# zqs01/ASR_chinese_e2e

Measured on AMD Instinct MI355X. Metric: training throughput (utterances/s; frames/s = x T), AISHELL-1-shaped 80-mel T=500, higher is better.
Workload: dtype bf16; 1 GPU; configs[2]: joint CTC/attention (lambda=0.3) encoder-decoder, bf16, per-GPU batch 32, T=500, F=80, V=4232, 6 layers, d_model 512, 8x64 heads, ff 1024, dropout 0.0, fwd+loss+CER+bwd+clip+Noam/Adam per step, eager launches; global_batch=32, seq_len=500, parallelism=dp1

## Files before the change

### asr_chinese_e2e_amd/Models/transformer_official.py

```python
import contextlib
import math

import numpy as np
import torch

from .. import engine as E
from .. import kernels as K
from ..Bases import BaseConfig, BaseModel
from ..Utils import Pack

SOS_ID, EOS_ID, PAD_ID = 2, 3, 0
PE_MAXLEN = 5000
CLIP_NORM = 5.0


def mwer_settings(weight, nbest, beam, frame_topk, blank_skip):
    try:
        ok = not isinstance(weight, (bool, str)) and math.isfinite(float(weight)) and float(weight) >= 0.0
    except (TypeError, ValueError):
        ok = False
    if not ok:
        raise ValueError(f"mwer_weight={weight!r}: a finite number >= 0 (0 = no MWER term)")
    for name, v in (("mwer_nbest", nbest), ("mwer_beam", beam), ("mwer_frame_topk", frame_topk)):
        if isinstance(v, bool) or not isinstance(v, (int, np.integer)):
# ... 676 lines not shown
            al = self._align_lists(ctc_logits(), wave_len, ids, alignable=ok, confidence=confidence)
            for o, a in zip(out, al):
                o["tokens"] = a["tokens"]
                if confidence is not None:
                    o["confidence"] = a["confidence"]
        return out

    def _ctc_cer(self, logits, wave_len, labels32, lab_len):
        ids, lens = K.ctc_greedy_decode(logits, wave_len, PAD_ID)
        return self._cer_ids(ids, labels32, hyp_len=lens, ref_len=lab_len)

    def train_step(self, input, loss_scale=1.0, count_hook=None):
        eng, x, wave_len, prep = self._prepare(input, training=self.training)
        B, T, _ = x.shape
        lam = self.ctc_weight
        ys_in, ys_out, labels32, dec_len, lab_len, n_valid = prep
        pending = count_hook(n_valid, B) if count_hook is not None else None
        zero, self._zero_lazy = (self._flat.g if getattr(self, "_zero_lazy", False) else None), False
        eng.refresh_transposes(zero=zero)
        enc, ecache = self.encode(eng, x, wave_len, training=True)
        batch_div = None
        if pending is not None:
            n_valid, batch_div = pending.wait()
        row_nll = nll = None
        d_enc = None
        pg = None
        ctc_done = None
        ctc_scale = dict(grad_scale=lam * loss_scale, grad_scale_div=batch_div) if batch_div is not None else dict(grad_scale=lam * loss_scale / float(B))
        ctc_async = (self.use_decoder and self.use_ctc and eng._aux_active() and not eng.deterministic)
        if self.use_decoder:
            cross_len, Tk = self._cross(eng, input, wave_len, T)
        if ctc_async:
            eng.decoder_kv_async(prep, enc, B, T, Tk)
            nll, d_enc, ctc_done = eng.ctc_branch_async(enc, wave_len, labels32, lab_len, B, T, **ctc_scale)
        if self.use_decoder:
            pred, dcache = eng.decoder_fwd(prep, enc, cross_len, B, T, Tk)
            ids = torch.empty(ys_out.shape, dtype=torch.int32, device=pred.device) if self.cer_in_iterate else None
            w_ce = (1.0 - lam) if self.use_ctc else 1.0
            row_nll, dpred = K.xent_fwd_bwd(pred, ys_out.reshape(-1), n_valid, PAD_ID, smoothing=self.label_smoothing, grad_scale=w_ce * loss_scale, dlogits=pred,
                                            argmax=ids)
            if ids is not None:
                pg = (ids, ys_out)
        if self.use_ctc and not ctc_async:
            path = torch.empty(B, T, dtype=torch.int32, device=enc.device) if (self.cer_in_iterate and not self.use_decoder) else None
            mwer = {}
            if self.mwer_weight > 0.0:
                mwer = dict(mwer_grad_scale=self.mwer_weight * loss_scale / (1.0 if batch_div is not None else float(B)))
            nll, d_enc = eng.ctc_fwd_bwd(enc, wave_len, labels32, lab_len, B, T, best_path=path, **ctc_scale, **mwer)
            if path is not None:
                def score():
                    ids, lens = K.ctc_collapse(path, wave_len, PAD_ID)
                    return self._cer_ids(ids, labels32, hyp_len=lens, ref_len=lab_len)
                pg = self._cer_beside_backward(eng, score, (path, wave_len, labels32, lab_len), inline=lambda: (score(), None))
        if self.use_decoder:
            if d_enc is None:
                d_enc = torch.zeros_like(enc)
            eng.decoder_bwd(dcache, dpred, d_enc, d_enc_ready=ctc_done)
            if pg is not None:
                pg = self._cer_beside_backward(eng, lambda: self._cer_ids(ids, ys_out), pg, inline=lambda: pg)
        eng.encoder_bwd(ecache, d_enc)
        loss = K.loss_combine(row_nll, n_valid, nll, (1.0 - lam) if self.use_ctc else 1.0, lam)
        self._mwer_mean = None
        if self.mwer_weight > 0.0 and self.use_ctc and not ctc_async:
            risk = eng.last_mwer[4]
            self._mwer_mean = risk.sum() / (batch_div[0] if batch_div is not None else float(B))
            loss = loss.clone()
            loss[0] += self.mwer_weight * self._mwer_mean
        return loss, pg

    def mwer_risk(self, input, nbest=None, beam_size=None, frame_topk=None, blank_skip=None):
        d = self._mwer
        _, m = mwer_settings(0.0, d["nbest"] if nbest is None else nbest, d["beam"] if beam_size is None else beam_size,
                             d["frame_topk"] if frame_topk is None else frame_topk, blank_skip)
        if blank_skip is None:
            m["thr"] = d["thr"]
        if self.use_decoder or not self.use_ctc:
            raise ValueError("mwer_risk needs the CTC-only model (TransformerCTC)")
        eng = self._ensure_engine(input.wave.device)
        was_training, eng.training = eng.training, False
        try:
            with torch.no_grad():
                out = self.forward(input)
        finally:
            eng.training = was_training
        logits = out.ctc_logits.contiguous()
        B, T, V = logits.shape
        wave_len = input.wave_len.to(torch.int32).contiguous()
        prep = K.dec_preprocess(input.tgt_for_input.contiguous(), SOS_ID, EOS_ID)
        labels32, lab_len = prep[2], prep[4]
        vals, ids, blank_lp = K.ctc_frame_topk(logits.view(B * T, V), min(m["frame_topk"], V), PAD_ID)
        search_len = wave_len
        if m["thr"] is not None:
            vals, ids, blank_lp, search_len, _ = K.ctc_blank_skip_compact(vals, ids, blank_lp, wave_len, m["thr"], B, T)
        Lh = min(T, K.MWER_MAX_LEN, 2 * labels32.shape[1] + 8)
        tok, ln, _ = K.ctc_prefix_beam(vals, ids, blank_lp, search_len, B, T, m["beam"], m["nbest"], PAD_ID, max_len=Lh)
        res = K.ctc_mwer(logits, wave_len, tok, ln, labels32, lab_len, blank=PAD_ID, want_grad=False)
        tok, ln, err, post, risk = (t.cpu().tolist() for t in (tok, ln, res["err"], res["post"], res["risk"]))
        return [{"risk": risk[b], "errors": [err[b][r] for r in range(m["nbest"]) if ln[b][r] >= 0],
                 "posteriors": [post[b][r] for r in range(m["nbest"]) if ln[b][r] >= 0],
                 "nbest": [tok[b][r][:min(ln[b][r], Lh)] for r in range(m["nbest"]) if ln[b][r] >= 0]} for b in range(B)]

    def iterate(self, input, optimizer=None, is_train=True):
        if optimizer is None or not is_train:
            with torch.no_grad():
                output = self.forward(input)
                return self.cal_metrics(output, input), None
        if self._ema_active:
            raise RuntimeError("iterate(is_train=True) inside ema_weights(): the parameters are swapped with their average")
        self._ensure_engine(input.wave.device)
        optimizer.zero_grad()
        if getattr(optimizer, "fused_step", None) is None or not getattr(optimizer, "keeps_grad_views", False):
            self._grads_checked = False
        self.zero_flat_grads()
        loss, pg = self.train_step(input)
# ... 59 lines not shown
```

### asr_chinese_e2e_amd/_lib.py

```python
import ctypes
import os
from ctypes import c_char_p, c_float, c_int, c_size_t, c_uint32, c_void_p

import torch

_HERE = os.path.dirname(os.path.abspath(__file__))
LIB_PATH = os.environ.get("ASR_HIP_LIB") or os.path.join(_HERE, "libasr_hip.so")

ASR_F32, ASR_BF16 = 0, 1
ACT_NONE, ACT_RELU, ACT_RELU_MASK = 0, 1, 2
ABI_VERSION = 10
DROP_PRE, DROP_POST = 1, 2
SPEED_TILE = 1024
RESAMPLE_TILE = 1024
REVERB_TILE, REVERB_CHUNK, REVERB_MAX_TAPS = 1024, 256, 8192
REVERB_FFT_N, REVERB_FFT_MAX_TAPS = 4096, 65536
NOISE_MIX_TILE = 4096
VAD_CTX_MAX = 1024
ALIGN_LONG_MAX_LABELS = 8192
SPECAUG_MAX_RANGES = 8
KWS_MAX_LEN, KWS_MAX_KEYWORDS, KWS_MAX_CAP = 16, 65536, 64
EDIT_LDS_DIR_BYTES, EDIT_MAX_REF = 98304, 16384
EDIT_COR, EDIT_SUB, EDIT_DEL, EDIT_INS = 0, 1, 2, 3
NBEST_MAX_N, NBEST_MAX_LEN, NBEST_MAX_ALTS, NBEST_EPS = 64, 256, 8, -1
RESCORE_MAX_N, RESCORE_MAX_K, RESCORE_MAX_G, RESCORE_MAX_U = 64, 8, 65536, 1 << 20
MWER_MAX_N, MWER_MAX_LEN, MWER_ABSENT, MWER_LONG = 16, 255, 1, 2
STREAM_OPEN = 0x3fffffff

P, I, F, Z, U = c_void_p, c_int, c_float, c_size_t, c_uint32

class TnProblem(ctypes.Structure):
    _fields_ = [("dY", P), ("X", P), ("dW", P), ("dbias", P), ("M", I), ("N", I), ("K", I), ("ldy", I), ("ldx", I), ("ldw", I)]


TN_GROUP_MAX = 8


class LnReduceItem(ctypes.Structure):
    _fields_ = [("ws", P), ("dgamma", P), ("dbeta", P), ("dbias", P), ("rows", I)]


LN_REDUCE_MAX = 16


class DecLayerPlan(ctypes.Structure):
    _fields_ = ([(n, I) for n in ("B", "To", "T", "d", "H", "dk", "ff")] + [("drop_p", F), ("seed", U * 5), ("ld_kv_c_T", I)] +
                [(n, P) for n in ("dec_len", "cross_len",
                                  "w_qkv_s", "w_fc_s", "w_q_c", "w_fc_c", "w_1", "w_2",
                                  "b_qkv_s", "b_fc_s", "b_q_c", "b_fc_c", "b_1", "b_2",
                                  "g_s", "be_s", "g_c", "be_c", "g_f", "be_f",
                                  "w_kv_c_T", "x_in",
                                  "qkv_s", "ctx_s", "a_s", "y_s", "lse_s", "rstd_s",
                                  "q_c", "kv_c", "kv_ready_event",
                                  "ctx_c", "a_c", "y_c", "lse_c", "rstd_c",
                                  "h", "o", "y_f", "rstd_f",
                                  "dz_f", "g_o", "g_h", "dx_f",
                                  "dz_c", "g_ac", "g_qc", "g_kvc", "dx_c",
                                  "dz_s", "g_as", "g_qkv", "dx_s",
                                  "dctx", "gb_2", "gb_fc_c", "gb_fc_s",
                                  "part_f", "part_c", "part_s", "delta")] +
                [("delta_bytes", Z), ("d_enc", P), ("wgrad_stream", P), ("aux_cus", I), ("ld_kv_c", I), ("kv_dgrad_cols", I), ("g_kv_group", P), ("ctx_s_lo", P), ("ctx_c_lo", P),
                 ("w_kv_c", P), ("g_enc_x", P), ("T_enc", I)])

SIGNATURES = {
    "asr_abi_version": (I, []),
    "asr_last_error": (I, [c_char_p, Z]),
    "asr_stream_fork": (I, [P, P]),
    "asr_stream_arm": (I, [P, P]),
    "asr_stream_arm_pending": (I, []),
    "asr_stream_create": (I, [I, P]),
    "asr_set_option": (I, [c_char_p, I, P]),
    "asr_get_deterministic": (I, []),
    "asr_set_deterministic": (I, [I]),
    "asr_add_ln_fwd": (I, [P, P, P, P, P, P, P, P, P, I, I, I, F, U, I, I, P]),
    "asr_add_ln_slots_fwd": (I, [P, P, P, P, P, P, P, P, I, I, I, I, I, P]),
    "asr_add_ln_bwd_workspace_bytes": (Z, [I, I]),
    "asr_add_ln_bwd": (I, [P, P, P, P, P, P, P, P, P, P, P, P, Z, I, I, I, F, U, I, I, P]),
    "asr_add_ln_bwd_reduce_batched": (I, [P, I, I, P]),
    "asr_sdpa_fwd": (I, [P, P, P, P, P, P, I, I, I, I, I, I, I, I, I, I, I, F, F, U, P, I, P]),
    "asr_sdpa_bwd_workspace_bytes": (Z, [I, I, I, I, I, I, I, I]),
    "asr_sdpa_bwd": (I, [P, P, P, P, P, P, P, Z, P, P, P, P, I, I, I, I, I, I, I, I, I, I, I, F, F, U, P, I, P]),
    "asr_sdpa_chunk_fwd": (I, [P, P, P, P, P, P, I, I, I, I, I, I, I, I, I, I, I, F, F, U, P, I, P]),
    "asr_sdpa_chunk_bwd_workspace_bytes": (Z, [I, I, I, I, I, I, I, I]),
    "asr_sdpa_chunk_bwd": (I, [P, P, P, P, P, P, P, Z, P, P, P, P, I, I, I, I, I, I, I, I, I, I, I, F, F, U, P, I, P]),
    "asr_dropout_mask": (I, [P, I, I, F, U, P]),
    "asr_sdpa_dropout_mask": (I, [P, I, I, I, I, F, U, P]),
    "asr_ctc_workspace_bytes": (Z, [I, I, I]),
    "asr_ctc_fwd_bwd": (I, [P, P, P, P, P, P, I, I, I, I, I, I, F, P, I, P, P, Z, I, P]),
    "asr_ctc_align_workspace_bytes": (Z, [I, I, I]),
    "asr_ctc_align": (I, [P, P, P, P, P, P, P, P, I, I, I, I, I, I, P, Z, I, P]),
    "asr_ctc_greedy_decode": (I, [P, P, P, P, I, I, I, I, I, I, P]),
    "asr_ctc_frame_argmax": (I, [P, P, P, I, I, I, I, I, I, P]),
    "asr_ctc_collapse": (I, [P, P, P, I, I, I, P]),
    "asr_decode_attn": (I, [P, P, P, P, P, I, I, I, I, I, I, I, I, I, I, I, F, I, P]),
    "asr_logsoftmax_topk": (I, [P, P, P, I, I, I, I, I, P]),
# ... 196 lines not shown
```

### asr_chinese_e2e_amd/csrc/ln.hip

```cpp
#include <stdlib.h>

#include "asr_common.h"

namespace {

constexpr int LN_WAVES = 4;
#ifndef LN_UNROLL
#define LN_UNROLL 2
#endif

template <typename T> struct Pack8;
template <> struct Pack8<bf16_t> { bf16x8 v; };
template <> struct Pack8<float> { f32x4 a, b; };
__device__ __forceinline__ void fetch8(const bf16_t* p, Pack8<bf16_t>& r) { r.v = *(const bf16x8*)p; }
__device__ __forceinline__ void fetch8(const float* p, Pack8<float>& r) { r.a = *(const f32x4*)p; r.b = *(const f32x4*)(p + 4); }
__device__ __forceinline__ void unpack8(const Pack8<bf16_t>& r, float* v) {
#pragma unroll
    for (int i = 0; i < 8; ++i) v[i] = (float)r.v[i];
}
__device__ __forceinline__ void unpack8(const Pack8<float>& r, float* v) {
#pragma unroll
    for (int i = 0; i < 4; ++i) { v[i] = r.a[i]; v[4 + i] = r.b[i]; }
}

template <typename T, int N, bool VEC8> struct RowSlice {
    struct Raw {
        Pack8<T> p[VEC8 ? N / 8 : 1];
        T s[VEC8 ? 1 : N];
    };
    static __device__ __forceinline__ void fetch(const T* p, int d, int lane, Raw& r) {
        if constexpr (VEC8) {
#pragma unroll
            for (int c = 0; c < N / 8; ++c) fetch8(p + c * 512 + lane * 8, r.p[c]);
        } else {
#pragma unroll
            for (int k = 0; k < N; ++k) {
                const int col = k * 64 + lane;
                r.s[k] = p[col < d ? col : 0];
            }
        }
    }
    static __device__ __forceinline__ void unpack(const Raw& r, int d, int lane, float (&v)[N]) {
        if constexpr (VEC8) {
#pragma unroll
            for (int c = 0; c < N / 8; ++c) unpack8(r.p[c], &v[c * 8]);
        } else {
#pragma unroll
            for (int k = 0; k < N; ++k) v[k] = (k * 64 + lane < d) ? to_f32<T>(r.s[k]) : 0.f;
        }
    }
    static __device__ __forceinline__ void load(const T* p, int d, int lane, float (&v)[N]) {
        if constexpr (VEC8) {
#pragma unroll
// ... 317 lines not shown
            case 2: LN_BWD(16, true); break;
            case 3: LN_BWD(24, true); break;
            default: LN_BWD(32, true); break;
        }
    } else {
        const int nk = ceil_div(d, 64);
        if (nk <= 1) LN_BWD(1, false);
        else if (nk <= 2) LN_BWD(2, false);
        else if (nk <= 4) LN_BWD(4, false);
        else if (nk <= 8) LN_BWD(8, false);
        else if (nk <= 16) LN_BWD(16, false);
        else LN_BWD(32, false);
    }
#undef LN_BWD
}

extern "C" int asr_add_ln_bwd(const void* dy, const void* dy2, const void* xhat, const float* rstd,
                              const float* gamma, const int32_t* lens, void* dz, void* dx, float* dgamma,
                              float* dbeta, float* dbias, void* ws, size_t ws_bytes, int B, int T,
                              int d, float drop_p, uint32_t drop_seed, int drop_mode, int dtype, void* stream) {
    if (!dy || !xhat || !rstd || !gamma || !dz || !ws || (!dgamma != !dbeta)) ASR_FAIL(ASR_EINVAL, "asr_add_ln_bwd: null pointer");
    if (B <= 0 || T <= 0 || d <= 0 || d > 2048) ASR_FAIL(ASR_EINVAL, "asr_add_ln_bwd: bad shape B=%d T=%d d=%d", B, T, d);
    const int rows = B * T;
    if (ws_bytes < asr_add_ln_bwd_workspace_bytes(rows, d)) ASR_FAIL(ASR_EWORKSPACE, "asr_add_ln_bwd: workspace %zu < %zu", ws_bytes, asr_add_ln_bwd_workspace_bytes(rows, d));
    if (dtype != ASR_F32 && dtype != ASR_BF16) ASR_FAIL(ASR_EDTYPE, "asr_add_ln_bwd: dtype %d", dtype);
    if (drop_p < 0.f || drop_p >= 1.f || (drop_p > 0.f && drop_mode != 1 && drop_mode != 2) || (drop_p > 0.f && (d & 1)))
        ASR_FAIL(ASR_EINVAL, "asr_add_ln_bwd: bad dropout p=%f mode=%d", drop_p, drop_mode);
    const int mode = drop_p > 0.f ? drop_mode : 0;
    if (mode == 1 && !dx) ASR_FAIL(ASR_EINVAL, "asr_add_ln_bwd: pre-residual dropout needs the dx output");
    hipStream_t st = (hipStream_t)stream;
    const uint32_t thr = drop_thr16(drop_p);
    const float ds = 1.f / (1.f - drop_p);
#define LN_BWD_D(TT, MODE) launch_ln_bwd<TT, MODE>(dy, dy2, xhat, rstd, gamma, lens, dz, dx, (float*)ws, rows, T, d, drop_seed, thr, ds, st)
    if (dtype == ASR_F32) { if (mode == 0) LN_BWD_D(float, 0); else if (mode == 1) LN_BWD_D(float, 1); else LN_BWD_D(float, 2); }
    else { if (mode == 0) LN_BWD_D(bf16_t, 0); else if (mode == 1) LN_BWD_D(bf16_t, 1); else LN_BWD_D(bf16_t, 2); }
#undef LN_BWD_D
    const int P = ln_grid(rows);
    const int ncols = dbias ? 3 * d : 2 * d;
    if (dgamma) {
        const int fsplit = 4;
        colsum_finalize_kernel<<<dim3(ceil_div(ncols, 32), (P >= 256 * fsplit && !asr_deterministic()) ? fsplit : 1), 1024, 0, st>>>((const float*)ws, P, (size_t)3 * d, ncols, d, dgamma, dbeta, dbias, 1);
    }
    ASR_CHECK_LAUNCH("asr_add_ln_bwd");
    return ASR_OK;
}

namespace {
struct LnReduceBatch {
    const float* part[ASR_LN_REDUCE_MAX];
    float* dgamma[ASR_LN_REDUCE_MAX];
    float* dbeta[ASR_LN_REDUCE_MAX];
    float* dbias[ASR_LN_REDUCE_MAX];
    int P[ASR_LN_REDUCE_MAX];
};
__global__ __launch_bounds__(1024) void ln_reduce_batched_kernel(const LnReduceBatch bt, int d) {
    __shared__ float red[32][33];
    const int it = blockIdx.z, P = bt.P[it];
    const float* __restrict__ part = bt.part[it];
    const int ncols = bt.dbias[it] ? 3 * d : 2 * d;
    const int cg = threadIdx.x & 31, pg = threadIdx.x >> 5;
    const int col = blockIdx.x * 32 + cg;
    const int ns = P >= 1024 ? (int)gridDim.y : 1;
    if (blockIdx.x * 32 >= ncols || (int)blockIdx.y >= ns) return;
    const int per = (P + ns - 1) / ns, pbeg = blockIdx.y * per, pend = min(P, pbeg + per);
    const size_t pstride = (size_t)3 * d;
    float s = 0.f;
    if (col < ncols) {
        int p = pbeg + pg;
        for (; p + 7 * 32 < pend; p += 8 * 32) {
            float v[8];
#pragma unroll
            for (int u = 0; u < 8; ++u) v[u] = part[(size_t)(p + u * 32) * pstride + col];
#pragma unroll
            for (int u = 0; u < 8; ++u) s += v[u];
        }
        for (; p < pend; p += 32) s += part[(size_t)p * pstride + col];
    }
    red[pg][cg] = s;
    __syncthreads();
    if (pg == 0 && col < ncols) {
        float t = 0.f;
#pragma unroll
        for (int i = 0; i < 32; ++i) t += red[i][cg];
        const int k = col / d, c = col - k * d;
        float* out = k == 0 ? bt.dgamma[it] : (k == 1 ? bt.dbeta[it] : bt.dbias[it]);
        if (ns > 1) atomicAdd(out + c, t);
        else out[c] += t;
    }
}
}

extern "C" int asr_add_ln_bwd_reduce_batched(const asr_ln_reduce_item* items, int n, int d, void* stream) {
    if (!items || n <= 0 || n > ASR_LN_REDUCE_MAX) ASR_FAIL(ASR_EINVAL, "asr_add_ln_bwd_reduce_batched: 1..%d items per call (got %d)", ASR_LN_REDUCE_MAX, n);
    if (d <= 0 || d > 2048) ASR_FAIL(ASR_EINVAL, "asr_add_ln_bwd_reduce_batched: bad d=%d", d);
    LnReduceBatch bt;
    memset(&bt, 0, sizeof(bt));
    for (int i = 0; i < n; ++i) {
        if (!items[i].ws || !items[i].dgamma || !items[i].dbeta || items[i].rows <= 0) ASR_FAIL(ASR_EINVAL, "asr_add_ln_bwd_reduce_batched: bad item %d", i);
        bt.part[i] = (const float*)items[i].ws;
        bt.dgamma[i] = items[i].dgamma;
        bt.dbeta[i] = items[i].dbeta;
        bt.dbias[i] = items[i].dbias;
        bt.P[i] = ln_grid(items[i].rows);
    }
    ln_reduce_batched_kernel<<<dim3(ceil_div(3 * d, 32), asr_deterministic() ? 1 : 4, n), 1024, 0, (hipStream_t)stream>>>(bt, d);
    ASR_CHECK_LAUNCH("asr_add_ln_bwd_reduce_batched");
    return ASR_OK;
}
```

### asr_chinese_e2e_amd/engine.py

```python
import math
import os

import torch

import collections
import ctypes

from . import _lib
from . import kernels as K
from ._lib import ACT_NONE, ACT_RELU, ACT_RELU_MASK

ALIGN = 64


def positional_encoding(max_len, d_model):
    pe = torch.zeros(max_len, d_model)
    pos = torch.arange(0, max_len).unsqueeze(1).float()
    w = torch.exp(torch.arange(0, d_model, 2).float() * -(math.log(10000.0) / d_model))
    pe[:, 0::2] = torch.sin(pos * w)
    pe[:, 1::2] = torch.cos(pos * w)
    return pe.unsqueeze(0)


class FlatParams:
# ... 973 lines not shown
                cross.kv.dgrad(t["g_kvc"], out=d_enc, accumulate=True)
            self._wgrad(ffn.w2, t["g_o"] if drop else t["dz_f"], t["h"])
            self._wgrad(ffn.w1, t["g_h"], t["y_c"], bias_from=t["g_h"])
            self._wgrad(cross.fc, t["g_ac"] if drop else t["dz_c"], t["ctx_c"])
            self._wgrad(cross.q, t["g_qc"], t["y_s"], bias_from=t["g_qc"])
            if not own_kv:
                self._wgrad(cross.kv, t["g_kvc"], enc, bias_from=t["g_kvc"])
            elif grp is not None:
                g = bufs["g_kv_all"][:, c0:c1]
                self._wgrad(self.kv_all.rows(c0, c1), g, src, bias_from=g)
            self._wgrad(slf.fc, t["g_as"] if drop else t["dz_s"], t["ctx_s"])
            self._wgrad(slf.qkv, t["g_qkv"], t["x_in"], bias_from=t["g_qkv"])
            self._ln_pending += [(t["part_f"], ffn.ln.gg, ffn.ln.gb, ffn.w2.gb, M), (t["part_c"], cross.ln.gg, cross.ln.gb, cross.fc.gb, M),
                                 (t["part_s"], slf.ln.gg, slf.ln.gb, slf.fc.gb, M)]
            dy, dy2 = t["dx_s"], t["dz_s"]
            self._ready(f"decoder.layer_stack.{i}.slf_attn.w_qs.weight")
            self._arm_covers_pending = False
        return dy, dy2

    def decoder_fwd(self, prep, enc, cross_len, B, T, Tk=None):
        ys_in, ys_out, labels32, dec_len, lab_len, n_valid = prep
        To = ys_in.shape[1]
        Tk = T if Tk is None else Tk
        pe_, se_ = self._drop(2)
        x = K.embed_pe_fwd(ys_in.reshape(-1), self.emb32, self.pe, self.d ** -0.5, B, To, self.dtype, drop_p=pe_, drop_seed=se_)
        cache = dict(B=B, T=T, To=To, ys_in=ys_in, layers=[], drop=(pe_, se_))
        if self._dec_exec_ok(B, To, T):
            x, bufs = self._dec_exec_fwd(x, enc, dec_len, cross_len, B, To, T, Tk)
            cache.update(exec_bufs=bufs, enc=enc, keep=(dec_len, cross_len))
            pred = self.prj.fwd(x)
            cache["x_last"] = x
            return pred, cache
        kv_pre = [None] * self.L
        kv_rows = T if Tk < T else None
        src = K.rows_gather(enc, B, T, Tk) if kv_rows else enc
        if self._aux_active():
            with _OnAux(self):
                for i, (slf, cross, ffn) in enumerate(self.dec):
                    kv = cross.kv.fwd(src)
                    e = torch.cuda.Event()
                    e.record(self.ctc_stream)
                    kv_pre[i] = (kv, e)
            self._keep += (enc, src)
            self._keep += [kv for kv, _ in kv_pre]
        for i, (slf, cross, ffn) in enumerate(self.dec):
            x1, c1 = self._attn_block_fwd(slf, x, x, B, To, To, dec_len, dec_len, dict(causal=True), cross=False, site=100 + 8 * i)
            x2, c2 = self._attn_block_fwd(cross, x1, src, B, To, Tk, cross_len, dec_len, {}, cross=True, site=102 + 8 * i, kv_pre=kv_pre[i], kv_rows=kv_rows)
            x, c3 = self._ffn_block_fwd(ffn, x2, B, To, dec_len, site=104 + 8 * i)
            cache["layers"].append((c1, c2, c3))
        pred = self.prj.fwd(x)
        cache["x_last"] = x
        return pred, cache

    def decoder_bwd(self, cache, dpred, d_enc, d_enc_ready=None):
        self._in_decoder = True
        self.wait_transposes()
        self._wgrad(self.prj, dpred, cache["x_last"])
        dy, dy2 = self.prj.dgrad(dpred), None
        if "exec_bufs" in cache:
            dy, dy2 = self._dec_exec_bwd(cache["exec_bufs"], dy, cache["enc"], d_enc, d_enc_ready)
        else:
            for i in reversed(range(self.L)):
                slf, cross, ffn = self.dec[i]
                c1, c2, c3 = cache["layers"][i]
                dx, dz = self._ffn_block_bwd(ffn, c3, dy, dy2)
                if d_enc_ready is not None:
                    torch.cuda.current_stream().wait_event(d_enc_ready)
                    d_enc_ready = None
                dx, dz = self._attn_block_bwd(cross, c2, dx, dz, d_kv_src=d_enc)
                dx, dz = self._attn_block_bwd(slf, c1, dx, dz)
                dy, dy2 = dx, dz
                self._ready(f"decoder.layer_stack.{i}.slf_attn.w_qs.weight")
        ids_flat, dyc, dy2c = cache["ys_in"].reshape(-1), dy.contiguous(), (dy2.contiguous() if dy2 is not None else None)
        self.flush_wgrads()
        if self.overlap_wgrad:
            self._disarm()
            self._fork(self.side)
            with _OnSide(self._side_handle):
                K.embed_bwd(ids_flat, dyc, self.gemb, self.d ** -0.5, drop_p=cache["drop"][0], drop_seed=cache["drop"][1], dy2=dy2c)
            self._keep += (ids_flat, dyc) + ((dy2c,) if dy2c is not None else ())
        else:
            K.embed_bwd(ids_flat, dyc, self.gemb, self.d ** -0.5, drop_p=cache["drop"][0], drop_seed=cache["drop"][1], dy2=dy2c)
        if self._aux_active():
            torch.cuda.current_stream().wait_stream(self.ctc_stream)
        self._in_decoder = False
        self._ready("decoder.tgt_word_emb.weight")
        if self.use_ctc:
            self._ready("ctc_lo.weight")
```

### asr_chinese_e2e_amd/kernels.py

```python
import math
import threading
import ctypes

import numpy as np
import torch

from . import _lib
from ._lib import ASR_BF16, ASR_F32, ACT_NONE, ACT_RELU, LN_REDUCE_MAX, TN_GROUP_MAX, LnReduceItem, TnProblem, check
from ._lib import fast as lib

_DT = {torch.float32: ASR_F32, torch.bfloat16: ASR_BF16}


def _dt(t):
    try:
        return _DT[t.dtype]
    except KeyError:
        raise TypeError(f"unsupported dtype {t.dtype} (float32 or bfloat16)")


def _p(t):
    if t is None:
        return None
    if not t.is_cuda:
# ... 110 lines not shown
    d = x.shape[-1]
    assert x.is_contiguous() and x.numel() == B * T * d
    if res is not None:
        assert res.is_contiguous() and res.shape == x.shape and res.dtype == x.dtype
    _chk_f32(gamma, beta, pe)
    _chk_i32(lens)
    assert gamma.numel() == d and beta.numel() == d
    if pe is not None:
        assert pe.shape[-1] == d and pe.shape[-2] >= T
    if lens is not None:
        assert lens.numel() == B
    y = torch.empty_like(x) if y is None else y
    xhat = torch.empty_like(x) if xhat is None else xhat
    rstd = torch.empty(B * T, dtype=torch.float32, device=x.device) if rstd is None else rstd
    nb = (3 + (res is not None)) * x.numel() * x.element_size()
    timed("add_ln_fwd", 0.0, lambda: check(
        lib.asr_add_ln_fwd(_p(x), _p(res), _p(gamma), _p(beta), _p(pe), _p(lens), _p(y), _p(xhat), _p(rstd),
                           B, T, d, float(drop_p), int(drop_seed) & 0xFFFFFFFF, int(drop_mode), _dt(x), _stream()), "asr_add_ln_fwd"), nb)
    return y, xhat, rstd


def add_ln_bwd(dy, dy2, xhat, rstd, gamma, lens, dgamma, dbeta, dbias, B, T, ws, dz=None, drop_p=0.0, drop_seed=0, drop_mode=0,
               partials=None):
    d = dy.shape[-1]
    assert dy.is_contiguous() and xhat.is_contiguous() and dy.numel() == B * T * d == xhat.numel()
    assert xhat.dtype == dy.dtype and (dy2 is None or (dy2.dtype == dy.dtype and dy2.is_contiguous() and dy2.numel() == dy.numel()))
    _chk_f32(rstd, gamma, dgamma, dbeta, dbias)
    _chk_i32(lens)
    assert rstd.numel() == B * T and dgamma.numel() == d and dbeta.numel() == d and (dbias is None or dbias.numel() == d)
    dz = torch.empty_like(dy) if dz is None else dz
    dx = torch.empty_like(dy) if (drop_p > 0 and drop_mode == 1) else None
    nbytes = lib.asr_add_ln_bwd_workspace_bytes(B * T, d)
    if partials is not None:
        assert partials.dtype == torch.uint8 and partials.numel() >= nbytes
        w, dgamma, dbeta = partials, None, None
    else:
        w = ws.get(nbytes)
    nb = (3 + (dy2 is not None) + (dx is not None)) * dy.numel() * dy.element_size()
    timed("add_ln_bwd", 0.0, lambda: check(
        lib.asr_add_ln_bwd(_p(dy), _p(dy2), _p(xhat), _p(rstd), _p(gamma), _p(lens), _p(dz), _p(dx), _p(dgamma), _p(dbeta),
                           _p(dbias), _p(w), w.numel(), B, T, d, float(drop_p), int(drop_seed) & 0xFFFFFFFF, int(drop_mode),
                           _dt(dy), _stream()), "asr_add_ln_bwd"), nb)
    return dz, (dx if dx is not None else dz)


def add_ln_bwd_workspace_bytes(rows, d):
    return lib.asr_add_ln_bwd_workspace_bytes(rows, d)


def add_ln_bwd_reduce_batched(items, d):
    for i in range(0, len(items), LN_REDUCE_MAX):
        chunk = items[i:i + LN_REDUCE_MAX]
        arr = (LnReduceItem * len(chunk))()
        for q, (part, dg, db, dbias, rows) in zip(arr, chunk):
            _chk_f32(dg, db, dbias)
            assert dg.numel() == d and db.numel() == d and (dbias is None or dbias.numel() == d)
            assert part.numel() >= lib.asr_add_ln_bwd_workspace_bytes(rows, d)
            q.ws, q.dgamma, q.dbeta, q.dbias, q.rows = _p(part), _p(dg), _p(db), _p(dbias), rows
        check(lib.asr_add_ln_bwd_reduce_batched(ctypes.addressof(arr), len(chunk), d, _stream()), "asr_add_ln_bwd_reduce_batched")


def _strided_rows(t, H, dk):
    assert t.dim() == 2 and t.stride(1) == 1 and t.shape[1] == H * dk
    return t.stride(0)


def _sdpa_entries(name):
    return (getattr(lib, name + "_fwd"), name + "_fwd"), (getattr(lib, name + "_bwd"), name + "_bwd"), getattr(lib, name + "_bwd_workspace_bytes")


_SDPA_PLAIN, _SDPA_CHUNK = _sdpa_entries("asr_sdpa"), _sdpa_entries("asr_sdpa_chunk")


def _sdpa_mask(causal, window, chunk, left_chunks):
    if chunk > 0:
        assert not causal and window < 0, "a chunk mask replaces causal / window"
        return *_SDPA_CHUNK, int(chunk), int(left_chunks)
    return *_SDPA_PLAIN, int(causal), int(window)


def sdpa_fwd(q, k, v, k_len, B, H, Tq, Tk, dk, causal=False, window=-1, scale=None, o=None, lse=None, drop_p=0.0, drop_seed=0, o_lo=None,
             chunk=0, left_chunks=-1):
    ldq, ldk, ldv = _strided_rows(q, H, dk), _strided_rows(k, H, dk), _strided_rows(v, H, dk)
    assert q.shape[0] == B * Tq and k.shape[0] == B * Tk and v.shape[0] == B * Tk
    assert q.dtype == k.dtype == v.dtype
    _chk_i32(k_len)
    assert k_len is None or k_len.numel() == B
    o = torch.empty(B * Tq, H * dk, dtype=q.dtype, device=q.device) if o is None else o
    ldo = _strided_rows(o, H, dk)
    lse = torch.empty(B, H, Tq, dtype=torch.float32, device=q.device) if lse is None else lse
    assert o_lo is None or (o_lo.dtype == o.dtype == torch.bfloat16 and o_lo.shape == o.shape and o_lo.stride() == o.stride())
    scale = float(dk) ** -0.5 if scale is None else float(scale)
    e = q.element_size()
    (fwd, name), _, _, a, b = _sdpa_mask(causal, window, chunk, left_chunks)
    timed("sdpa_fwd", 4.0 * B * H * Tq * Tk * dk, lambda: check(
        fwd(_p(q), _p(k), _p(v), _p(o), _p(lse), _p(k_len), B, H, Tq, Tk, dk, ldq, ldk, ldv, ldo,
            a, b, scale, float(drop_p), int(drop_seed) & 0xFFFFFFFF, _p(o_lo), _dt(q), _stream()), name),
          2.0 * B * H * (Tq + Tk) * dk * e)
    return o, lse


def sdpa_bwd(q, k, v, o, do, lse, k_len, B, H, Tq, Tk, dk, dq, dk_, dv, causal=False, window=-1, scale=None, delta=None,
             drop_p=0.0, drop_seed=0, o_lo=None, chunk=0, left_chunks=-1):
    ldq, ldk, ldv, ldo = (_strided_rows(t, H, dk) for t in (q, k, v, o))
    assert _strided_rows(do, H, dk) == ldo and _strided_rows(dq, H, dk) == ldq
    assert _strided_rows(dk_, H, dk) == ldk and _strided_rows(dv, H, dk) == ldv
    assert q.dtype == k.dtype == v.dtype == o.dtype == do.dtype == dq.dtype == dk_.dtype == dv.dtype
    _chk_i32(k_len)
    _chk_f32(lse)
    assert o_lo is None or (o_lo.dtype == o.dtype == torch.bfloat16 and o_lo.shape == o.shape and o_lo.stride() == o.stride())
    _, (bwd, name), workspace_bytes, a, b = _sdpa_mask(causal, window, chunk, left_chunks)
# ... 1528 lines not shown
```

### include/asr_hip.h

```cpp
#ifndef ASR_HIP_H
#define ASR_HIP_H

#include <stddef.h>
#include <stdint.h>

#ifdef __cplusplus
extern "C" {
#endif

#define ASR_ABI_VERSION 10

typedef enum { ASR_F32 = 0, ASR_BF16 = 1 } asr_dtype_t;

#define ASR_OK 0
#define ASR_EINVAL (-1)
#define ASR_EDTYPE (-2)
#define ASR_EWORKSPACE (-3)
#define ASR_EHIP (-4)

#define ASR_ACT_NONE 0
#define ASR_ACT_RELU 1
#define ASR_ACT_RELU_MASK 2

int asr_abi_version(void);
int asr_last_error(char* buf, size_t n);
int asr_stream_fork(void* from_stream, void* to_stream);
int asr_stream_arm(void* from_stream, void* to_stream);
int asr_stream_arm_pending(void);
int asr_stream_create(int priority, void** out_stream);
int asr_set_option(const char* name, int value, int* previous);
int asr_get_deterministic(void);
int asr_set_deterministic(int on);

#define ASR_DROP_PRE 1
#define ASR_DROP_POST 2
int asr_add_ln_fwd(const void* x, const void* res, const float* gamma, const float* beta,
                   const float* pe, const int32_t* lens, void* y, void* xhat, float* rstd,
                   int B, int T, int d, float drop_p, uint32_t drop_seed, int drop_mode, int dtype,
                   void* stream);

int asr_add_ln_slots_fwd(void* x, const float* gamma, const float* beta, const float* pe, const int32_t* pe_off,
                         const int32_t* lens, void* y, float* rstd, int slots, int T, int d, int pe_rows, int dtype, void* stream);

size_t asr_add_ln_bwd_workspace_bytes(int rows, int d);
int asr_add_ln_bwd(const void* dy, const void* dy2, const void* xhat, const float* rstd,
                   const float* gamma, const int32_t* lens, void* dz, void* dx, float* dgamma,
                   float* dbeta, float* dbias, void* ws, size_t ws_bytes, int B, int T, int d,
                   float drop_p, uint32_t drop_seed, int drop_mode, int dtype, void* stream);
#define ASR_LN_REDUCE_MAX 16
typedef struct asr_ln_reduce_item {
    const void* ws;
    float* dgamma;
    float* dbeta;
    float* dbias;
    int rows;
} asr_ln_reduce_item;
int asr_add_ln_bwd_reduce_batched(const asr_ln_reduce_item* items, int n, int d, void* stream);

int asr_sdpa_fwd(const void* q, const void* k, const void* v, void* o, float* lse,
                 const int32_t* k_len, int B, int H, int Tq, int Tk, int dk, int ldq, int ldk,
                 int ldv, int ldo, int causal, int window, float scale, float drop_p,
                 uint32_t drop_seed, void* o_lo, int dtype, void* stream);

size_t asr_sdpa_bwd_workspace_bytes(int B, int H, int Tq, int Tk, int dk, int causal, int window, int dtype);
int asr_sdpa_bwd(const void* q, const void* k, const void* v, const void* o, const void* d_o,
                 const float* lse, float* delta, size_t delta_bytes, void* dq, void* dk_, void* dv,
                 const int32_t* k_len, int B, int H, int Tq, int Tk, int dk, int ldq, int ldk,
                 int ldv, int ldo, int causal, int window, float scale, float drop_p,
                 uint32_t drop_seed, const void* o_lo, int dtype, void* stream);

int asr_sdpa_chunk_fwd(const void* q, const void* k, const void* v, void* o, float* lse,
                       const int32_t* k_len, int B, int H, int Tq, int Tk, int dk, int ldq, int ldk,
                       int ldv, int ldo, int chunk, int left_chunks, float scale, float drop_p,
                       uint32_t drop_seed, void* o_lo, int dtype, void* stream);
size_t asr_sdpa_chunk_bwd_workspace_bytes(int B, int H, int Tq, int Tk, int dk, int chunk, int left_chunks, int dtype);
int asr_sdpa_chunk_bwd(const void* q, const void* k, const void* v, const void* o, const void* d_o,
                       const float* lse, float* delta, size_t delta_bytes, void* dq, void* dk_, void* dv,
                       const int32_t* k_len, int B, int H, int Tq, int Tk, int dk, int ldq, int ldk,
                       int ldv, int ldo, int chunk, int left_chunks, float scale, float drop_p,
                       uint32_t drop_seed, const void* o_lo, int dtype, void* stream);

int asr_dropout_mask(uint8_t* mask, int rows, int cols, float drop_p, uint32_t drop_seed, void* stream);
int asr_sdpa_dropout_mask(uint8_t* mask, int B, int H, int Tq, int Tk, float drop_p, uint32_t drop_seed, void* stream);

size_t asr_ctc_workspace_bytes(int B, int T, int Lmax);
int asr_ctc_fwd_bwd(const void* logits, void* dlogits, const int32_t* in_len,
                    const int32_t* labels, const int32_t* lab_len, float* nll, int B, int T, int V, int ld,
                    int Lmax, int blank, float grad_scale, const float* grad_scale_div, int zero_infinity,
                    int32_t* best_path, void* ws, size_t ws_bytes, int dtype, void* stream);

size_t asr_ctc_align_workspace_bytes(int B, int T, int Lmax);
int asr_ctc_align(const void* logits, const int32_t* in_len, const int32_t* labels, const int32_t* lab_len, int32_t* path,
                  int32_t* spans, float* token_logp, float* score, int B, int T, int V, int ld, int Lmax, int blank, void* ws,
                  size_t ws_bytes, int dtype, void* stream);

int asr_ctc_greedy_decode(const void* logits, const int32_t* in_len, int32_t* out_ids,
                          int32_t* out_len, int B, int T, int V, int ld, int blank, int dtype, void* stream);
int asr_ctc_frame_argmax(const void* logits, const int32_t* in_len, int32_t* path, int B, int T, int V, int ld, int blank,
                         int dtype, void* stream);
int asr_ctc_collapse(int32_t* ids, const int32_t* in_len, int32_t* out_len, int B, int T, int blank, void* stream);

int asr_ctc_frame_topk(const void* logits, float* vals, int32_t* ids, float* blank_lp, int R, int V, int ld, int k,
                       int blank, int dtype, void* stream);
size_t asr_ctc_prefix_beam_workspace_bytes(int B, int T, int beam);
int asr_ctc_prefix_beam(const float* vals, const int32_t* ids, const float* blank_lp, const int32_t* in_len, void* ws, size_t ws_bytes,
                        int32_t* out_tok, int32_t* out_len, float* out_score, int B, int T, int k, int beam, int nbest, int Lcap,
                        int blank, void* stream);
size_t asr_ctc_prefix_beam_state_bytes(int B, int beam);
// ... 386 lines not shown
```

Before: 7209 utterances/s.

## Overlap LN reduce flush and loss combine with decoder backward on side stream

Moves the batched LayerNorm gamma/beta reduction flush and the loss-combine kernel onto the side stream during decoder backward, so they overlap with the main-stream backward instead of running serially afterwards. The batched reduce kernel now accepts a per-item width d, doubles the batch capacity to 32 items, and sorts items by partial count. It also drops the split-P atomicAdd path, so each item is reduced by a single block column over all partials. This cuts launches and serialization, but large-P items lose the intra-item parallelism they had before.

```diff
diff --git a/asr_chinese_e2e_amd/Models/transformer_official.py b/asr_chinese_e2e_amd/Models/transformer_official.py
--- a/asr_chinese_e2e_amd/Models/transformer_official.py
+++ b/asr_chinese_e2e_amd/Models/transformer_official.py
@@ -752,14 +752,18 @@
                     ids, lens = K.ctc_collapse(path, wave_len, PAD_ID)
                     return self._cer_ids(ids, labels32, hyp_len=lens, ref_len=lab_len)
                 pg = self._cer_beside_backward(eng, score, (path, wave_len, labels32, lab_len), inline=lambda: (score(), None))
+        loss_box = []
+
+        def combine():
+            return K.loss_combine(row_nll, n_valid, nll, (1.0 - lam) if self.use_ctc else 1.0, lam)
         if self.use_decoder:
             if d_enc is None:
                 d_enc = torch.zeros_like(enc)
-            eng.decoder_bwd(dcache, dpred, d_enc, d_enc_ready=ctc_done)
+            eng.decoder_bwd(dcache, dpred, d_enc, d_enc_ready=ctc_done, beside=lambda: loss_box.append(combine()))
             if pg is not None:
                 pg = self._cer_beside_backward(eng, lambda: self._cer_ids(ids, ys_out), pg, inline=lambda: pg)
         eng.encoder_bwd(ecache, d_enc)
-        loss = K.loss_combine(row_nll, n_valid, nll, (1.0 - lam) if self.use_ctc else 1.0, lam)
+        loss = loss_box[0] if loss_box else combine()
         self._mwer_mean = None
         if self.mwer_weight > 0.0 and self.use_ctc and not ctc_async:
             risk = eng.last_mwer[4]
diff --git a/asr_chinese_e2e_amd/_lib.py b/asr_chinese_e2e_amd/_lib.py
--- a/asr_chinese_e2e_amd/_lib.py
+++ b/asr_chinese_e2e_amd/_lib.py
@@ -37,10 +37,10 @@
 
 
 class LnReduceItem(ctypes.Structure):
-    _fields_ = [("ws", P), ("dgamma", P), ("dbeta", P), ("dbias", P), ("rows", I)]
-
-
-LN_REDUCE_MAX = 16
+    _fields_ = [("ws", P), ("dgamma", P), ("dbeta", P), ("dbias", P), ("rows", I), ("d", I)]
+
+
+LN_REDUCE_MAX = 32
 
 
 class DecLayerPlan(ctypes.Structure):
diff --git a/asr_chinese_e2e_amd/csrc/ln.hip b/asr_chinese_e2e_amd/csrc/ln.hip
--- a/asr_chinese_e2e_amd/csrc/ln.hip
+++ b/asr_chinese_e2e_amd/csrc/ln.hip
@@ -1,4 +1,6 @@
 #include <stdlib.h>
+
+#include <algorithm>
 
 #include "asr_common.h"
 
@@ -422,29 +424,28 @@
     float* dbeta[ASR_LN_REDUCE_MAX];
     float* dbias[ASR_LN_REDUCE_MAX];
     int P[ASR_LN_REDUCE_MAX];
+    int d[ASR_LN_REDUCE_MAX];
 };
-__global__ __launch_bounds__(1024) void ln_reduce_batched_kernel(const LnReduceBatch bt, int d) {
+__global__ __launch_bounds__(1024) void ln_reduce_batched_kernel(const LnReduceBatch bt) {
     __shared__ float red[32][33];
-    const int it = blockIdx.z, P = bt.P[it];
+    const int it = blockIdx.y, P = bt.P[it], d = bt.d[it];
     const float* __restrict__ part = bt.part[it];
     const int ncols = bt.dbias[it] ? 3 * d : 2 * d;
     const int cg = threadIdx.x & 31, pg = threadIdx.x >> 5;
     const int col = blockIdx.x * 32 + cg;
-    const int ns = P >= 1024 ? (int)gridDim.y : 1;
-    if (blockIdx.x * 32 >= ncols || (int)blockIdx.y >= ns) return;
-    const int per = (P + ns - 1) / ns, pbeg = blockIdx.y * per, pend = min(P, pbeg + per);
+    if (blockIdx.x * 32 >= ncols) return;
     const size_t pstride = (size_t)3 * d;
     float s = 0.f;
     if (col < ncols) {
-        int p = pbeg + pg;
-        for (; p + 7 * 32 < pend; p += 8 * 32) {
+        int p = pg;
+        for (; p + 7 * 32 < P; p += 8 * 32) {
             float v[8];
 #pragma unroll
             for (int u = 0; u < 8; ++u) v[u] = part[(size_t)(p + u * 32) * pstride + col];
 #pragma unroll
             for (int u = 0; u < 8; ++u) s += v[u];
         }
-        for (; p < pend; p += 32) s += part[(size_t)p * pstride + col];
+        for (; p < P; p += 32) s += part[(size_t)p * pstride + col];
     }
     red[pg][cg] = s;
     __syncthreads();
@@ -454,8 +455,7 @@
         for (int i = 0; i < 32; ++i) t += red[i][cg];
         const int k = col / d, c = col - k * d;
         float* out = k == 0 ? bt.dgamma[it] : (k == 1 ? bt.dbeta[it] : bt.dbias[it]);
-        if (ns > 1) atomicAdd(out + c, t);
-        else out[c] += t;
+        out[c] += t;
     }
 }
 }
@@ -465,15 +465,26 @@
     if (d <= 0 || d > 2048) ASR_FAIL(ASR_EINVAL, "asr_add_ln_bwd_reduce_batched: bad d=%d", d);
     LnReduceBatch bt;
     memset(&bt, 0, sizeof(bt));
+    int dmax = 0;
     for (int i = 0; i < n; ++i) {
-        if (!items[i].ws || !items[i].dgamma || !items[i].dbeta || items[i].rows <= 0) ASR_FAIL(ASR_EINVAL, "asr_add_ln_bwd_reduce_batched: bad item %d", i);
-        bt.part[i] = (const float*)items[i].ws;
-        bt.dgamma[i] = items[i].dgamma;
-        bt.dbeta[i] = items[i].dbeta;
-        bt.dbias[i] = items[i].dbias;
-        bt.P[i] = ln_grid(items[i].rows);
-    }
-    ln_reduce_batched_kernel<<<dim3(ceil_div(3 * d, 32), asr_deterministic() ? 1 : 4, n), 1024, 0, (hipStream_t)stream>>>(bt, d);
+        const int di = items[i].d ? items[i].d : d;
+        if (!items[i].ws || !items[i].dgamma || !items[i].dbeta || items[i].rows <= 0 || di <= 0 || di > 2048)
+            ASR_FAIL(ASR_EINVAL, "asr_add_ln_bwd_reduce_batched: bad item %d", i);
+        dmax = di > dmax ? di : dmax;
+    }
+    int order[ASR_LN_REDUCE_MAX];
+    for (int i = 0; i < n; ++i) order[i] = i;
+    std::stable_sort(order, order + n, [&](int a, int b) { return ln_grid(items[a].rows) > ln_grid(items[b].rows); });
+    for (int i = 0; i < n; ++i) {
+        const asr_ln_reduce_item& q = items[order[i]];
+        bt.part[i] = (const float*)q.ws;
+        bt.dgamma[i] = q.dgamma;
+        bt.dbeta[i] = q.dbeta;
+        bt.dbias[i] = q.dbias;
+        bt.P[i] = ln_grid(q.rows);
+        bt.d[i] = q.d ? q.d : d;
+    }
+    ln_reduce_batched_kernel<<<dim3(ceil_div(3 * dmax, 32), n), 1024, 0, (hipStream_t)stream>>>(bt);
     ASR_CHECK_LAUNCH("asr_add_ln_bwd_reduce_batched");
     return ASR_OK;
 }
diff --git a/asr_chinese_e2e_amd/engine.py b/asr_chinese_e2e_amd/engine.py
--- a/asr_chinese_e2e_amd/engine.py
+++ b/asr_chinese_e2e_amd/engine.py
@@ -1049,7 +1049,7 @@
         cache["x_last"] = x
         return pred, cache
 
-    def decoder_bwd(self, cache, dpred, d_enc, d_enc_ready=None):
+    def decoder_bwd(self, cache, dpred, d_enc, d_enc_ready=None, beside=None):
         self._in_decoder = True
         self.wait_transposes()
         self._wgrad(self.prj, dpred, cache["x_last"])
@@ -1075,9 +1075,15 @@
             self._fork(self.side)
             with _OnSide(self._side_handle):
                 K.embed_bwd(ids_flat, dyc, self.gemb, self.d ** -0.5, drop_p=cache["drop"][0], drop_seed=cache["drop"][1], dy2=dy2c)
+                if self.grad_ready is None:
+                    self.flush_ln_reduce()
+                if beside is not None:
+                    beside()
             self._keep += (ids_flat, dyc) + ((dy2c,) if dy2c is not None else ())
         else:
             K.embed_bwd(ids_flat, dyc, self.gemb, self.d ** -0.5, drop_p=cache["drop"][0], drop_seed=cache["drop"][1], dy2=dy2c)
+            if beside is not None:
+                beside()
         if self._aux_active():
             torch.cuda.current_stream().wait_stream(self.ctc_stream)
         self._in_decoder = False
diff --git a/asr_chinese_e2e_amd/kernels.py b/asr_chinese_e2e_amd/kernels.py
--- a/asr_chinese_e2e_amd/kernels.py
+++ b/asr_chinese_e2e_amd/kernels.py
@@ -186,11 +186,12 @@
     for i in range(0, len(items), LN_REDUCE_MAX):
         chunk = items[i:i + LN_REDUCE_MAX]
         arr = (LnReduceItem * len(chunk))()
-        for q, (part, dg, db, dbias, rows) in zip(arr, chunk):
+        for q, (part, dg, db, dbias, rows, *own) in zip(arr, chunk):
+            di = own[0] if own else d
             _chk_f32(dg, db, dbias)
-            assert dg.numel() == d and db.numel() == d and (dbias is None or dbias.numel() == d)
-            assert part.numel() >= lib.asr_add_ln_bwd_workspace_bytes(rows, d)
-            q.ws, q.dgamma, q.dbeta, q.dbias, q.rows = _p(part), _p(dg), _p(db), _p(dbias), rows
+            assert dg.numel() == di and db.numel() == di and (dbias is None or dbias.numel() == di)
+            assert part.numel() >= lib.asr_add_ln_bwd_workspace_bytes(rows, di)
+            q.ws, q.dgamma, q.dbeta, q.dbias, q.rows, q.d = _p(part), _p(dg), _p(db), _p(dbias), rows, di
         check(lib.asr_add_ln_bwd_reduce_batched(ctypes.addressof(arr), len(chunk), d, _stream()), "asr_add_ln_bwd_reduce_batched")
 
 
diff --git a/include/asr_hip.h b/include/asr_hip.h
--- a/include/asr_hip.h
+++ b/include/asr_hip.h
@@ -47,13 +47,14 @@
                    const float* gamma, const int32_t* lens, void* dz, void* dx, float* dgamma,
                    float* dbeta, float* dbias, void* ws, size_t ws_bytes, int B, int T, int d,
                    float drop_p, uint32_t drop_seed, int drop_mode, int dtype, void* stream);
-#define ASR_LN_REDUCE_MAX 16
+#define ASR_LN_REDUCE_MAX 32
 typedef struct asr_ln_reduce_item {
     const void* ws;
     float* dgamma;
     float* dbeta;
     float* dbias;
     int rows;
+    int d;
 } asr_ln_reduce_item;
 int asr_add_ln_bwd_reduce_batched(const asr_ln_reduce_item* items, int n, int d, void* stream);
 
```

New measurement: 7197 utterances/s. Within noise of the previous version (-0.2%).
